# fnzhan/Neural-Gauge-Fields

Measured on AMD Instinct MI355X. Metric: Mray/sec (800x800 lego-style frame, 192 samples/ray), higher is better.
Workload: dtype f32; 1 GPU; TriPlane 800x800 frame, S=192, preset R1 (seeded random planes 256^2, dense density preset), gauge on, white_bg; samples_per_ray=192, bake_density=1, bake_color=1, launcher=none (single process)

## Files before the change

include/ngf.h:

```cpp
#ifndef NGF_H
#define NGF_H
#include <stdint.h>

#ifdef __cplusplus
extern "C" {
#endif

#define NGF_ABI_VERSION 5

enum { NGF_OK = 0, NGF_E_ARG = 1, NGF_E_HIP = 2, NGF_E_UNSUPPORTED = 3,
       NGF_E_STALE = 4  };
enum { NGF_MODEL_TRIPLANE = 0, NGF_MODEL_INFOINV = 1 };

enum {
    NGF_F_BAKE_DENSITY = 1,
    NGF_F_NO_FOLD = 4,
    NGF_F_SPLIT_BF16 = 8,
    NGF_F_BAKE_COLOR = 2
};

typedef struct ngf_field_desc {
    int32_t model;
    int32_t flags;
    int32_t plane_c;
// ... 159 lines not shown
int ngf_uv_texture_eval(const ngf_uv *m, const float *uv, const float *view, int32_t view_stride, int64_t n, int32_t flags, float *out,
                        void *hip_stream);
int ngf_uv_render(const ngf_uv *m, const float *campos_host, const float *raydir, const float *bg_host,
                  const float *jitter_u, int64_t n_rays, int32_t n_samples, float *color, float *transmittance,
                  float *dbg_sigma, float *dbg_col, uint64_t *stats, void *hip_stream);

int ngf_uv_render_batch(const ngf_uv *m, const float *campos_dev, const float *raydir, const float *bg_dev, const float *jitter_u,
                        int32_t n_cams, int64_t rays_per_cam, int32_t n_samples, float *color, float *transmittance,
                        float *dbg_sigma, float *dbg_col, uint64_t *stats, void *hip_stream);

int ngf_debug_set(const char *name, int32_t value);
int32_t ngf_debug_get(const char *name);
int ngf_debug_dirty_lds(void *hip_stream);
int ngf_debug_xcd_histogram(unsigned *out8, int32_t workgroups, void *hip_stream);
int ngf_debug_tile_plan(int64_t n, int32_t wide, int64_t resident, int32_t tail16, int64_t *seg_rays, int32_t *seg_shift);
#define NGF_UV_TRAIN_PARAMS (2 * NGF_UV_LAYERS)
typedef struct ngf_uv_train_desc {
    int32_t sphere;
    int32_t flags;
    const float *w[NGF_UV_LAYERS];
    const float *b[NGF_UV_LAYERS];
    int64_t max_rays;
    int32_t max_samples;
    int32_t pad_;
} ngf_uv_train_desc;
typedef struct ngf_uv_trainer ngf_uv_trainer;
int ngf_uv_trainer_create(const ngf_uv_train_desc *desc, ngf_uv_trainer **out, void *hip_stream);
int ngf_uv_trainer_destroy(ngf_uv_trainer *t);
int64_t ngf_uv_trainer_bytes(const ngf_uv_trainer *t);
int32_t ngf_sizeof_uv_train_desc(void);
// ... 23 lines not shown
```

neural-gauge-fields_amd/_lib.py:

```python
from __future__ import annotations

import ctypes as C
import os
import subprocess

_CSRC = os.path.join(os.path.dirname(os.path.abspath(__file__)), "csrc")
SO_PATH = os.path.join(_CSRC, "libngf_hip.so")
SO_PATH_EXP = os.path.join(_CSRC, "libngf_hip_exp.so")
_LIB = None
_LIBS = {}

MODEL_TRIPLANE, MODEL_INFOINV = 0, 1
F_BAKE_DENSITY = 1
F_BAKE_COLOR = 2
F_NO_FOLD = 4
F_SPLIT_BF16 = 8

SYMBOLS = ["ngf_field_create", "ngf_field_destroy", "ngf_field_render", "ngf_field_render_image", "ngf_field_decode_rgb", "ngf_field_march",
           "ngf_generate_rays", "ngf_generate_rays_dtu", "ngf_last_error", "ngf_abi_version", "ngf_field_bytes", "ngf_sizeof_field_desc",
           "ngf_uv_create", "ngf_uv_destroy", "ngf_uv_render", "ngf_uv_render_batch", "ngf_field_alpha", "ngf_field_ray_filter",
           "ngf_eval_workspace_bytes", "ngf_eval_frame_u8", "ngf_eval_depth_range", "ngf_eval_depth_colormap", "ngf_eval_mse",
           "ngf_eval_ssim", "ngf_trainer_create", "ngf_trainer_destroy", "ngf_trainer_bytes", "ngf_sizeof_train_desc", "ngf_train_backward", "ngf_train_backward2",
           "ngf_train_forward", "ngf_train_backward_grad", "ngf_train_get_grad", "ngf_train_get_active", "ngf_train_overflow_count", "ngf_train_adam", "ngf_train_adam_all", "ngf_train_adam_ext", "ngf_train_get_grads", "ngf_train_params_changed", "ngf_train_debug_sections", "ngf_resize_bilinear", "ngf_uv_set_texture", "ngf_uv_texture_edit", "ngf_field_alpha_mask_build", "ngf_pack_mask_bits", "ngf_debug_set", "ngf_debug_get", "ngf_debug_dirty_lds", "ngf_debug_xcd_histogram", "ngf_debug_tile_plan", "ngf_debug_tile_order", "ngf_planes_l1", "ngf_planes_l1_backward", "ngf_pool_trim", "ngf_pool_set_limit", "ngf_pool_bytes",
           "ngf_infoinv_trainer_create", "ngf_infoinv_trainer_destroy", "ngf_infoinv_trainer_bytes", "ngf_sizeof_infoinv_train_desc",
           "ngf_infoinv_train_forward", "ngf_infoinv_train_backward_grad", "ngf_infoinv_train_get_grads", "ngf_infoinv_train_params_changed",
           "ngf_infoinv_train_step_backward", "ngf_infoinv_train_set_moments", "ngf_infoinv_train_adam_all", "ngf_infoinv_train_get_grad",
           "ngf_infoinv_train_adam_ext",
           "ngf_uv_trainer_create", "ngf_uv_trainer_destroy", "ngf_uv_trainer_bytes", "ngf_sizeof_uv_train_desc", "ngf_uv_train_forward",
           "ngf_uv_train_backward", "ngf_uv_train_get_grads", "ngf_uv_train_params_changed", "ngf_uv_texture_eval"]


class FieldDesc(C.Structure):
    _fields_ = [
        ("model", C.c_int32), ("flags", C.c_int32), ("plane_c", C.c_int32), ("dens_dim", C.c_int32),
        ("plane", C.c_void_p * 3), ("plane_h", C.c_int32 * 3), ("plane_w", C.c_int32 * 3),
        ("gauge", C.c_void_p * 3), ("gauge_h", C.c_int32 * 3), ("gauge_w", C.c_int32 * 3),
        ("dens_w1", C.c_void_p), ("dens_b1", C.c_void_p), ("dens_w2", C.c_void_p),
        ("dens_b2", C.c_void_p), ("dens_w3", C.c_void_p), ("dens_b3", C.c_void_p),
# ... 70 lines not shown
        L.ngf_resize_bilinear.argtypes = [C.c_void_p, C.c_int32, C.c_int32, C.c_int32, C.c_void_p, C.c_int32, C.c_int32, C.c_void_p]
        L.ngf_eval_workspace_bytes.restype = C.c_int64
        L.ngf_eval_workspace_bytes.argtypes = [C.c_int32, C.c_int32, C.c_int32]
        L.ngf_eval_frame_u8.argtypes = [C.c_void_p, C.c_int64, C.c_void_p, C.c_void_p]
        L.ngf_eval_depth_range.argtypes = [C.c_void_p, C.c_int64, C.c_void_p, C.c_void_p, C.c_void_p]
        L.ngf_eval_depth_colormap.argtypes = [C.c_void_p, C.c_int64, C.c_void_p, C.c_void_p, C.c_void_p, C.c_void_p]
        L.ngf_eval_mse.argtypes = [C.c_void_p, C.c_void_p, C.c_int64, C.c_void_p, C.c_void_p, C.c_void_p]
        L.ngf_eval_ssim.argtypes = [C.c_void_p, C.c_void_p, C.c_int32, C.c_int32, C.c_double, C.c_int32, C.c_double, C.c_double,
                                    C.c_double, C.c_void_p, C.c_void_p, C.c_void_p, C.c_void_p]
        L.ngf_debug_set.argtypes = [C.c_char_p, C.c_int32]
        L.ngf_debug_get.argtypes = [C.c_char_p]
        L.ngf_debug_get.restype = C.c_int32
        L.ngf_debug_dirty_lds.argtypes = [C.c_void_p]
        L.ngf_debug_xcd_histogram.argtypes = [C.c_void_p, C.c_int32, C.c_void_p]
        L.ngf_debug_tile_plan.argtypes = [C.c_int64, C.c_int32, C.c_int64, C.c_int32, C.POINTER(C.c_int64), C.POINTER(C.c_int32)]
        L.ngf_pool_set_limit.argtypes = [C.c_int64]
        L.ngf_pool_bytes.argtypes = [C.c_int32]
        L.ngf_pool_bytes.restype = C.c_int64
        L.ngf_planes_l1.argtypes = [C.c_void_p, C.c_void_p, C.c_void_p, C.c_void_p, C.c_void_p]
        L.ngf_planes_l1_backward.argtypes = [C.c_void_p, C.c_void_p, C.c_void_p, C.c_void_p, C.c_void_p]
        L.ngf_debug_tile_order.argtypes = [C.c_void_p, C.c_int64, C.c_uint32, C.c_uint32, C.c_uint32, C.c_uint32, C.c_void_p]
        if L.ngf_abi_version() != 5 or L.ngf_sizeof_field_desc() != C.sizeof(FieldDesc):
            raise RuntimeError("libngf_hip.so ABI mismatch (version or ngf_field_desc layout)")
        _LIBS[path] = L
    return _LIBS[path]


class library:

    def __init__(self, which="exp"):
# ... 32 lines not shown
            check(L.ngf_debug_set(k.encode(), int(v)))
        return self

    def __exit__(self, *exc):
        L = lib()
        for k, v in self.old.items():
            L.ngf_debug_set(k.encode(), int(v))
        return False


def knobs_from_env():
    global _LIB
    if any(os.environ.get("NGF_" + k.upper()) not in (None, "", "-1") for k in ("waves", "nstep", "profile", "kernel", "stage")):
        _LIB = _load(SO_PATH_EXP)
    L = lib()
    for k in ("tile_w", "split", "waves", "nstep", "profile", "ablate", "uv_tiles", "kernel", "stage", "xcd", "grid", "tail", "ord_rows", "ord_px", "train_dwg"):
        v = os.environ.get("NGF_" + k.upper())
        check(L.ngf_debug_set(k.encode(), int(v) if v not in (None, "") else -1))
```

neural-gauge-fields_amd/csrc/ngf_device.hpp:

```cpp
#pragma once
#include <cstddef>
#include <type_traits>
#include <hip/hip_runtime.h>
#include <stdint.h>

typedef float f32x2 __attribute__((ext_vector_type(2)));
typedef float f32x4 __attribute__((ext_vector_type(4)));
typedef float f32x16 __attribute__((ext_vector_type(16)));

namespace ngf {

constexpr int kWave = 64;
constexpr int kRing = 128;
constexpr int kRecFloats = 8;
constexpr int kViewFeat = 16;

struct Tex {
    const float *p;
    int32_t W, H;
    int32_t stride;
    float fw, fh;
};

struct MaskVol {
// ... 19 lines not shown
    int32_t S, white_bg, mode, skip_rgb;
    int32_t tile_w;
    int32_t tile_shift;
    uint32_t seg_end[3];
    int32_t seg_shift[4];
    int64_t seg_ray0[4];
    int32_t xcd_queues;
    int32_t waves_active;
    uint32_t tiles;
    uint32_t ord_n;
    uint32_t ord_tpr;
    uint32_t ord_bw;
    uint32_t ord_bh;
    uint32_t queue_waves;
    int32_t ablate;
    float a0[3], a1[3], inv[3];
    float near_, far_, step, dscale, thr;
    Tex dens[3];
    Tex app[3];
    Tex gau[3];
    MaskVol mask;
    const float *basis_pack;
    const float *blob;
    int32_t blob_floats;
    float wd[48];
    float bd;
};

__device__ __forceinline__ int xcd_id() { return (int)(__builtin_amdgcn_s_getreg((3 << 11) | 20) & 7u); }

// ... 110 lines not shown
    b.wx1 = wx1; b.wy1 = wy1; b.in = in ? 1 : 0;
    wx0 = in ? wx0 : 0.0f;
    wx1 = in ? wx1 : 0.0f;
    wy0 = in ? wy0 : 0.0f;
    wy1 = in ? wy1 : 0.0f;
    b.cx = (int)cx + 1;
    b.cy = (int)cy + 1;
    b.idx = (int)__umul24((unsigned)b.cy, (unsigned)t.stride) + b.cx;
    b.w00 = wx0 * wy0;
    b.w10 = wx1 * wy0;
    b.w01 = wx0 * wy1;
    b.w11 = wx1 * wy1;
    return b;
}

template <typename T>
__device__ __forceinline__ const T *tex_at(const float *base, uint32_t float_index)
{
    return reinterpret_cast<const T *>(reinterpret_cast<const char *>(base) + (size_t)(uint32_t)(float_index * 4u));
}

__device__ __forceinline__ Bil bil_from_rec(int32_t idx, float wx1, float wy1, bool in)
{
    Bil b;
    b.idx = idx; b.cx = 0; b.cy = 0; b.wx1 = wx1; b.wy1 = wy1; b.in = in ? 1 : 0;
    float wx0 = 1.0f - wx1;
    float wy0 = 1.0f - wy1;
    wx0 = in ? wx0 : 0.0f;
    wx1 = in ? wx1 : 0.0f;
    wy0 = in ? wy0 : 0.0f;
// ... 138 lines not shown
```

neural-gauge-fields_amd/csrc/ngf_field.hip:

```cpp
#include <map>
#include <mutex>
#include <utility>

#include "ngf_host.hpp"
#include "ngf_infoinv.hpp"
#include "ngf_render.hpp"
#ifdef NGF_EXPERIMENTS
#include "ngf_render_pc.hpp"
#include "ngf_stage.hpp"
#endif
#include "ngf_train.hpp"

using namespace ngf;

static thread_local char g_err[512] = "";

int ngf::fail(int code, const char *fmt, ...)
{
    va_list ap;
    va_start(ap, fmt);
    vsnprintf(g_err, sizeof(g_err), fmt, ap);
    va_end(ap);
    return code;
}

static std::atomic<int> g_knob[ngf::KNOB_COUNT];
static const char *const g_knob_name[ngf::KNOB_COUNT] = {"tile_w", "split", "waves", "nstep", "profile", "ablate", "uv_tiles", "kernel", "stage", "poison", "grid", "xcd", "tail", "ord_rows", "ord_px", "train_dwg"};
static bool g_knob_init = [] { for (auto &k : g_knob) k.store(-1); return true; }();

int ngf::knob(int id) { return g_knob[id].load(std::memory_order_relaxed); }

hipError_t ngf::ensure_dynamic_lds(const void *kernel, size_t bytes)
{
    static std::mutex mu;
    static std::map<std::pair<int, const void *>, size_t> done;
    int dev = 0;
    hipError_t e = hipGetDevice(&dev);
    if (e != hipSuccess) return e;
    std::lock_guard<std::mutex> lock(mu);
    size_t &have = done[{dev, kernel}];
    if (have >= bytes && have != 0) return hipSuccess;
    e = hipFuncSetAttribute(kernel, hipFuncAttributeMaxDynamicSharedMemorySize, (int)bytes);
// ... 96 lines not shown
    mutable std::mutex use_mu;
    mutable std::vector<hipStream_t> streams;
    mutable std::atomic<void *> last_stream{(void *)(intptr_t)-1};
};

static inline void field_use(const ngf_field *f, hipStream_t st)
{
    if (f->last_stream.load(std::memory_order_relaxed) == (void *)st) return;
    std::lock_guard<std::mutex> lk(f->use_mu);
    bool known = false;
    for (hipStream_t s : f->streams) known |= s == st;
    if (!known) f->streams.push_back(st);
    f->last_stream.store((void *)st, std::memory_order_relaxed);
}

__global__ void pack_plane_kernel(const float *__restrict__ src, int H, int W, int c0, int nc, float *__restrict__ dst, int perm = 0)
{
    const size_t total = (size_t)(H + 2) * (W + 2) * nc;
    for (size_t i = (size_t)blockIdx.x * blockDim.x + threadIdx.x; i < total; i += (size_t)gridDim.x * blockDim.x) {
        const int c = (int)(i % nc);
        const size_t tx = i / nc;
        const int x = (int)(tx % (W + 2)), y = (int)(tx / (W + 2));
        float v = 0.0f;
        if (x >= 1 && x <= W && y >= 1 && y <= H) v = src[((size_t)(c0 + (perm ? infoinv_split_channel(c) : c)) * H + (y - 1)) * W + (x - 1)];
        dst[i] = v;
    }
}

__global__ void __launch_bounds__(256) mask_cells_kernel(const uint8_t *__restrict__ bits, int D, int H, int W, uint8_t *__restrict__ cells)
{
    ngf::MaskVol m{};
    m.bits = bits; m.D = D; m.H = H; m.W = W;
    const size_t total = (size_t)(D + 1) * (H + 1) * (W + 1);
    for (size_t i = (size_t)blockIdx.x * blockDim.x + threadIdx.x; i < total; i += (size_t)gridDim.x * blockDim.x) {
        const int x = (int)(i % (size_t)(W + 1)) - 1, y = (int)((i / (size_t)(W + 1)) % (size_t)(H + 1)) - 1, z = (int)(i / ((size_t)(W + 1) * (H + 1))) - 1;
        unsigned c = 0;
#pragma unroll
        for (int k = 0; k < 8; ++k) c |= (unsigned)ngf::mask_bit(m, z + (k >> 2), y + ((k >> 1) & 1), x + (k & 1)) << k;
        cells[i] = (uint8_t)c;
    }
}
// ... 21 lines not shown
{
    const int b = blockIdx.x * blockDim.x + threadIdx.x;
    if (b >= cD * cH * cW) return;
    const int X = b % cW, Y = (b / cW) % cH, Z = b / (cW * cH);
    unsigned acc = 0;
    for (int dz = -1; dz <= 1; ++dz)
        for (int dy = -1; dy <= 1; ++dy)
            for (int dx = -1; dx <= 1; ++dx) {
                const int x = X + dx, y = Y + dy, z = Z + dz;
                if (x >= 0 && x < cW && y >= 0 && y < cH && z >= 0 && z < cD) acc |= any[(z * cH + y) * cW + x];
            }
    clear[b] = acc ? 0 : 1;
}

__global__ void bake_density_kernel(const float *__restrict__ src, int H, int W, int nc, const float *__restrict__ wd,
                                    float *__restrict__ dst)
{
    const size_t total = (size_t)(H + 2) * (W + 2);
    for (size_t i = (size_t)blockIdx.x * blockDim.x + threadIdx.x; i < total; i += (size_t)gridDim.x * blockDim.x) {
        const int x = (int)(i % (W + 2)), y = (int)(i / (W + 2));
        double v = 0.0;
        if (x >= 1 && x <= W && y >= 1 && y <= H)
            for (int c = 0; c < nc; ++c) v += (double)wd[c] * (double)src[((size_t)c * H + (y - 1)) * W + (x - 1)];
        dst[i] = (float)v;
    }
}

__global__ void __launch_bounds__(256) bake_color_kernel(const float *__restrict__ src, int H, int W, int c0, int nc, const double *__restrict__ wp, int ldw,
                                                         float *__restrict__ dst)
{
    const size_t texels = (size_t)(H + 2) * (W + 2), plane = (size_t)H * W;
    const int lane = threadIdx.x & 63, w = __builtin_amdgcn_readfirstlane(threadIdx.x >> 6);
    const double *wr = wp + (size_t)(16 * w) * ldw;
    for (size_t t0 = (size_t)blockIdx.x * 64; t0 < texels; t0 += (size_t)gridDim.x * 64) {
        const size_t tx = t0 + lane;
        if (tx >= texels) continue;
        const int x = (int)(tx % (W + 2)), y = (int)(tx / (W + 2));
        const bool inside = x >= 1 && x <= W && y >= 1 && y <= H;
        const float *sp = src + ((size_t)c0 * H + (inside ? y - 1 : 0)) * W + (inside ? x - 1 : 0);
// ... 572 lines not shown
        return bail(fail(NGF_E_HIP, "uploading the MLP image failed"));
    A.blob = f->blob;
    A.blob_floats = (int)img.size();
    if (no_fold || split_ii) {
        if ((rc = alloc_f(&f->basis_pack, bpack.size(), f, st))) return bail(rc);
        if (hipMemcpyAsync(f->basis_pack, bpack.data(), bpack.size() * sizeof(float), hipMemcpyHostToDevice, st) != hipSuccess)
            return bail(fail(NGF_E_HIP, "uploading the packed basis matrix failed"));
        A.basis_pack = f->basis_pack;
    }
    if (tri) {
        for (int i = 0; i < 48; ++i) A.wd[i] = dw1[i];
        A.bd = db1[0];
    }

    NGF_CT("image upload");
    const int app_c = bake_c ? 64 : f->app;
    for (int p = 0; p < 3; ++p) {
        const int H = d->plane_h[p], W = d->plane_w[p];
        const size_t texels = (size_t)(H + 2) * (W + 2);
        const int dc = bake ? 1 : d->dens_dim;
        if (texels * (size_t)(app_c > 96 ? app_c : 96) * sizeof(float) >= ((size_t)1 << 32)) {
            return bail(fail(NGF_E_UNSUPPORTED, "plane %d: %d x %d texels do not fit a 4 GiB packed texture", p, H, W));
        }
        if ((rc = alloc_f(&f->tex[p], texels * dc, f, st)) || (rc = alloc_f(&f->tex[3 + p], texels * app_c, f, st))) return bail(rc);
        if (bake) bake_density_kernel<<<1024, 256, 0, st>>>(d->plane[p], H, W, d->dens_dim, d->dens_w1 + p * d->dens_dim, f->tex[p]);
        else pack_plane_kernel<<<2048, 256, 0, st>>>(d->plane[p], H, W, 0, d->dens_dim, f->tex[p]);
        if (bake_c) bake_color_kernel<<<2048, 256, 0, st>>>(d->plane[p], H, W, d->dens_dim, f->app, f->w1pd_tmp + (size_t)p * f->app, F, f->tex[3 + p]);
        else pack_plane_kernel<<<2048, 256, 0, st>>>(d->plane[p], H, W, d->dens_dim, f->app, f->tex[3 + p], tri ? 0 : 1);
        A.dens[p] = Tex{f->tex[p], W, H, W + 2, (float)(W - 1), (float)(H - 1)};
        A.app[p] = Tex{f->tex[3 + p], W, H, W + 2, (float)(W - 1), (float)(H - 1)};
        if (tri) {
            const int gh = d->gauge_h[p], gw = d->gauge_w[p];
            if ((rc = alloc_f(&f->tex[6 + p], (size_t)(gh + 2) * (gw + 2) * 2, f, st))) return bail(rc);
            pack_plane_kernel<<<256, 256, 0, st>>>(d->gauge[p], gh, gw, 0, 2, f->tex[6 + p]);
            A.gau[p] = Tex{f->tex[6 + p], gw, gh, gw + 2, (float)(gw - 1), (float)(gh - 1)};
        }
    }
    NGF_CT("texture allocs + launches");
    const bool launch_ok = hipGetLastError() == hipSuccess && hipStreamSynchronize(st) == hipSuccess;
    NGF_CT("sync (pack / bake kernels)");
    f->w1p_tmp = nullptr; f->w1pd_tmp = nullptr;
    if (!launch_ok) return bail(fail(NGF_E_HIP, "packing kernels failed"));

    for (int k = 0; k < 3; ++k) {
        A.a0[k] = d->aabb[k];
        A.a1[k] = d->aabb[3 + k];
        A.inv[k] = 2.0f / (d->aabb[3 + k] - d->aabb[k]);
    }
    A.near_ = d->near_; A.far_ = d->far_; A.step = d->step; A.dscale = d->distance_scale; A.thr = d->weight_thres;
// ... 164 lines not shown
    A.xcd_queues = knob(KNOB_XCD) > 0 ? 8 : 1;
    int64_t grid = tiles < f->num_cus ? tiles : f->num_cus;
    if (knob(KNOB_GRID) > 0 && grid > knob(KNOB_GRID)) grid = knob(KNOB_GRID);
    if (grid < 1) grid = 1;
    const int64_t per_wg = (tiles + grid - 1) / grid;
    A.waves_active = per_wg < waves ? (int)per_wg : waves;
    A.queue_waves = (uint32_t)grid;
    hipLaunchKernelGGL(k, dim3((unsigned)grid), dim3(threads), lds_bytes, st, A);
    HIP_TRY(hipGetLastError());
    return NGF_OK;
}

template <typename P>
static int launch_policy(const ngf_field *f, RenderArgs &A, hipStream_t st)
{
    const size_t lds = ((size_t)((A.blob_floats + 3) & ~3) + P::WAVES * wave_lds_floats<P>()) * sizeof(float);
    if (lds > 160 * 1024) return fail(NGF_E_ARG, "this waves-per-CU setting needs %zu bytes of LDS (> 160 KiB)", lds);
    constexpr int wide = P::INFOINV ? 16 : 8;
    using KP = decltype(&render_kernel<P, false>);
    if constexpr (P::NSTEP == 1 && P::PROD) return launch_render<KP>(render_kernel<P, false>, render_kernel<P, true>, render_kernel<P, true, false>, f, A, P::WAVES * kWave, lds, st, wide);
    else if constexpr (P::NSTEP == 1) return launch_render<KP>(render_kernel<P, false>, render_kernel<P, true>, nullptr, f, A, P::WAVES * kWave, lds, st, wide);
    else return launch_render<KP>(render_kernel<P, false>, nullptr, nullptr, f, A, P::WAVES * kWave, lds, st, wide);
}

#ifdef NGF_EXPERIMENTS
template <typename P, int NM, int NS, int TW>
static int launch_pc(const ngf_field *f, RenderArgs &A, hipStream_t st)
{
    const size_t lds = ((size_t)((A.blob_floats + 3) & ~3) + PcLds<NM>::TOTAL) * sizeof(float);
    if (lds > 160 * 1024) return fail(NGF_E_ARG, "the specialised kernel needs %zu bytes of LDS (> 160 KiB)", lds);
    const unsigned slot = f->next_counter.fetch_add(1) % kCounters;
    A.tile_counter = f->counters + (size_t)slot * kQueueHeads;
    HIP_TRY(hipMemsetAsync(A.tile_counter, 0, kQueueHeads * sizeof(unsigned), st));
    if (int rc = poison_lds(st)) return rc;
    A.xcd_queues = 1;
    A.tile_w = TW;
    A.tile_shift = TW == 8 ? 3 : 2;
    auto k = render_pc_kernel<P, NM, NS, TW>;
    HIP_TRY(ensure_dynamic_lds(reinterpret_cast<const void *>(k), lds));
    const int64_t tiles = (A.n + TW - 1) / TW;
    int64_t grid = (tiles + NM - 1) / NM;
    if (grid > f->num_cus) grid = f->num_cus;
    if (grid < 1) grid = 1;
// ... 175 lines not shown
    A.mode = mode ? 1 : 0;
    if (int rc = poison_lds(st)) return rc;
    int64_t grid = (n + 255) / 256;
    if (grid > 8 * (int64_t)f->num_cus) grid = 8 * (int64_t)f->num_cus;
    if (f->model == NGF_MODEL_INFOINV) {
        const size_t lds = (size_t)((A.blob_floats + 3) & ~3) * sizeof(float);
        if (grid > (int64_t)f->num_cus) grid = f->num_cus;
        if (f->flags & NGF_F_SPLIT_BF16) {
            HIP_TRY(ensure_dynamic_lds(reinterpret_cast<const void *>(alpha_kernel<InfoInvSplitPolicy>), lds));
            hipLaunchKernelGGL(alpha_kernel<InfoInvSplitPolicy>, dim3((unsigned)grid), dim3(256), lds, st, A, xyz, L, n, length, alpha);
        } else {
            HIP_TRY(ensure_dynamic_lds(reinterpret_cast<const void *>(alpha_kernel<InfoInvPolicy>), lds));
            hipLaunchKernelGGL(alpha_kernel<InfoInvPolicy>, dim3((unsigned)grid), dim3(256), lds, st, A, xyz, L, n, length, alpha);
        }
    } else if (f->flags & NGF_F_BAKE_DENSITY) {
        hipLaunchKernelGGL((alpha_kernel<TriPlanePolicy<true, false, 8, 1>>), dim3((unsigned)grid), dim3(256), 0, st, A, xyz, L, n, length, alpha);
    } else {
        hipLaunchKernelGGL((alpha_kernel<TriPlanePolicy<false, false, 8, 1>>), dim3((unsigned)grid), dim3(256), 0, st, A, xyz, L, n, length, alpha);
    }
    HIP_TRY(hipGetLastError());
    return NGF_OK;
}

extern "C" int ngf_field_alpha(const ngf_field *f, const float *xyz, int64_t n, int32_t mode, float length, float *alpha, void *hip_stream)
{
    if (!f || !xyz || !alpha) return fail(NGF_E_ARG, "ngf_field_alpha: null argument");
    if (n < 0) return fail(NGF_E_ARG, "ngf_field_alpha: n=%lld", (long long)n);
    if (n == 0) return NGF_OK;
    return launch_alpha(f, xyz, Lattice{nullptr, nullptr, nullptr, 0, 0, 0}, n, mode, length, alpha, (hipStream_t)hip_stream);
}

// ... 778 lines not shown
```

neural-gauge-fields_amd/csrc/ngf_host.hpp:

```cpp
#pragma once
#include <hip/hip_runtime.h>

#include <algorithm>
#include <atomic>
#include <cmath>
#include <cstdarg>
#include <chrono>
#include <cstdio>
#include <cstring>
#include <cstdlib>
#include <new>
#include <vector>

#include "../../include/ngf.h"

namespace ngf {

int fail(int code, const char *fmt, ...) __attribute__((format(printf, 2, 3)));

static constexpr int kCounters = 256;
static constexpr int kQueueHeads = 16;

enum Knob { KNOB_TILE_W = 0, KNOB_SPLIT, KNOB_WAVES, KNOB_NSTEP, KNOB_PROFILE, KNOB_ABLATE, KNOB_UV_TILES, KNOB_KERNEL, KNOB_STAGE, KNOB_POISON, KNOB_GRID, KNOB_XCD, KNOB_TAIL, KNOB_ORD_ROWS, KNOB_ORD_PX, KNOB_TRAIN_DWG, KNOB_COUNT };
int knob(int id);
hipError_t ensure_dynamic_lds(const void *kernel, size_t bytes);
constexpr unsigned kPoisonPattern = 0x7FC0DEADu;
int poison_lds(hipStream_t st);
int poison_alloc(void *p, size_t bytes, hipStream_t st);

}

#define HIP_TRY(expr)                                                                                        \
    do {                                                                                                     \
        hipError_t e_ = (expr);                                                                              \
        if (e_ != hipSuccess) return ngf::fail(NGF_E_HIP, "%s failed: %s", #expr, hipGetErrorString(e_));    \
    } while (0)

namespace ngf {
// ... 21 lines not shown
```

neural-gauge-fields_amd/csrc/ngf_render.hpp:

```cpp
#pragma once
#include <cstddef>
#include <type_traits>

#include "ngf_device.hpp"
#include "ngf_shade16.hpp"
#include "ngf_shade_bf16.hpp"

namespace ngf {


template <typename P> constexpr int wave_lds_floats() { return P::RING * kRecFloats + P::BATCH * 4 + P::VFEAT_FLOATS + P::STAGE_FLOATS; }

__device__ __forceinline__ void view_inputs(const float d[3], float v[16])
{
    v[0] = d[0]; v[1] = d[1]; v[2] = d[2];
#pragma unroll
    for (int k = 0; k < 3; ++k) {
        sincos_small(d[k], v[3 + 2 * k], v[9 + 2 * k]);
        sincos_small(d[k] * 2.0f, v[4 + 2 * k], v[10 + 2 * k]);
    }
    v[15] = 0.0f;
}

__device__ __forceinline__ void view_inputs_tile(const float d[3], float *dst, int seg, int K)
// ... 37 lines not shown
{
#pragma unroll
    for (int base = 0; base < F; base += 4) {
        float s, c;
        sincos_small(x * (float)(1 << base), s, c);
        sn[base] = s; cs[base] = c;
#pragma unroll
        for (int j = 1; j < 4 && base + j < F; ++j) {
            const float s2 = 2.0f * s * c, c2 = (c - s) * (c + s);
            s = s2; c = c2;
            sn[base + j] = s; cs[base + j] = c;
        }
    }
}

template <bool BAKED>
__device__ __forceinline__ float triplane_density_feature(const RenderArgs &A, const float t[6], Bil *cells = nullptr)
{
    float f = 0.0f;
#pragma unroll
    for (int p = 0; p < 3; ++p) {
        const Tex tx = karg_tex(offsetof(RenderArgs, dens) + p * sizeof(Tex));
        Bil b = bil_setup<BAKED>(t[2 * p], t[2 * p + 1], tx);
        if (cells) cells[p] = b;
        if (BAKED) {
            const float *q = tex_at<float>(tx.p, (uint32_t)b.idx), *q1 = tex_at<float>(tx.p, (uint32_t)(b.idx + tx.stride));
            f += bil_mix(b, q[0], q[1], q1[0], q1[1]);
        } else {
            const f32x4 *q00 = tex_at<f32x4>(tx.p, (uint32_t)b.idx * 16u);
            const f32x4 *q01 = tex_at<f32x4>(tx.p, (uint32_t)(b.idx + tx.stride) * 16u);
            float d00 = 0.0f, d10 = 0.0f, d01 = 0.0f, d11 = 0.0f;
            typedef const __attribute__((address_space(4))) float *kptr_t;
            kptr_t wdp = (kptr_t)((const __attribute__((address_space(4))) char *)__builtin_amdgcn_kernarg_segment_ptr() + offsetof(RenderArgs, wd)) + p * 16;
            asm volatile("" : "+s"(wdp));
#pragma unroll
            for (int q = 0; q < 4; ++q) {
                f32x4 v00 = q00[q], v10 = q00[4 + q], v01 = q01[q], v11 = q01[4 + q];
#pragma unroll
                for (int e = 0; e < 4; ++e) {
                    float w = wdp[4 * q + e];
                    d00 = fmaf(w, v00[e], d00);
                    d10 = fmaf(w, v10[e], d10);
                    d01 = fmaf(w, v01[e], d01);
                    d11 = fmaf(w, v11[e], d11);
                }
            }
            f += bil_mix(b, d00, d10, d01, d11);
        }
    }
    return f + A.bd;
}

template <bool MED3 = true>
__device__ __forceinline__ void triplane_gauge(const RenderArgs &A, const float x[3], int gauge_on, float t[6])
{
    const float u[3] = {x[0], x[1], x[0]}, v[3] = {x[1], x[2], x[2]};
    if (gauge_on) {
        float d[3][2];
#pragma unroll
        for (int p = 0; p < 3; ++p) {
            const Tex tx = karg_tex(offsetof(RenderArgs, gau) + p * sizeof(Tex));
            Bil b = bil_setup<MED3>(u[p], v[p], tx);
            const f32x2 *g = tex_at<f32x2>(tx.p, (uint32_t)b.idx * 2u), *g1 = tex_at<f32x2>(tx.p, (uint32_t)(b.idx + tx.stride) * 2u);
            f32x2 g00 = g[0], g10 = g[1], g01 = g1[0], g11 = g1[1];
            d[p][0] = bil_mix(b, g00[0], g10[0], g01[0], g11[0]);
            d[p][1] = bil_mix(b, g00[1], g10[1], g01[1], g11[1]);
        }
        t[0] = (u[0] + d[0][0]) + d[2][0];  t[1] = (v[0] + d[0][1]) + d[1][0];
        t[2] = (u[1] + d[1][0]) + d[0][1];  t[3] = (v[1] + d[1][1]) + d[2][1];
        t[4] = (u[2] + d[2][0]) + d[0][0];  t[5] = (v[2] + d[2][1]) + d[1][1];
    } else {
#pragma unroll
        for (int p = 0; p < 3; ++p) { t[2 * p] = u[p]; t[2 * p + 1] = v[p]; }
    }
}

template <bool BAKE_D, bool BAKE_C, int WAVES_, int NSTEP_, bool PROFILE_ = false>
struct TriPlanePolicy {
    static constexpr bool PROFILE = PROFILE_;
    static constexpr bool PROD = WAVES_ == 12 && NSTEP_ == 1 && !PROFILE_;
    static constexpr bool INFOINV = false;
    static constexpr bool MASK_SKIP = false;
    static constexpr bool STAGED = false;
    static constexpr int STAGE_FLOATS = 0;
    static constexpr int WAVES = WAVES_;
    static constexpr int NSTEP = NSTEP_;
    static constexpr int BATCH = kBatch16;
    static constexpr bool VLDS = WAVES_ <= 12;
    static constexpr int VFEAT_FLOATS = VLDS ? kWave * kViewFeat : 0;
    static constexpr int RING = NSTEP_ == 1 ? 128 : 256;
    static constexpr bool REC12 = WAVES_ == 12 && NSTEP_ == 1 && !PROFILE_;
    static constexpr bool GATHER_QUAD = BAKE_C;
    __device__ static __forceinline__ float sigma(const RenderArgs &A, const float *, bool valid, const float x[3], int, float t[6], Bil *cells = nullptr)
    {
        float tt[6];
        triplane_gauge<BAKE_D>(A, x, A.mode, tt);
        const float sg = softplus_shift(triplane_density_feature<BAKE_D>(A, tt, cells));
#pragma unroll
        for (int k = 0; k < 6; ++k) t[k] = valid ? tt[k] : 0.0f;
        return valid ? sg : 0.0f;
    }
    static constexpr bool VIEW_FOLD = VLDS;
    __device__ static __forceinline__ void fold_view(const float *smem, const float *vfeat, float *pre, int n_rays, int lane)
    {
        if constexpr (BAKE_C) view_fold16<MlpLayout16Baked::W1V / 64, MlpLayout16Baked::B1, 4>(per_pass16(smem), vfeat, pre, n_rays, lane);
        else view_fold16<MlpLayout16<48>::W1 / 64 + 3 * MlpLayout16<48>::QCH, MlpLayout16<48>::B1, MlpLayout16<48>::KT>(per_pass16(smem), vfeat, pre, n_rays, lane);
    }
    __device__ static __forceinline__ void fold_view_regs(const float *smem, const f32x4 v, float *pre, int n_rays, int lane)
    {
        if constexpr (BAKE_C) view_fold16_regs<MlpLayout16Baked::W1V / 64, MlpLayout16Baked::B1, 4>(per_pass16(smem), v, pre, n_rays, lane);
        else view_fold16_regs<MlpLayout16<48>::W1 / 64 + 3 * MlpLayout16<48>::QCH, MlpLayout16<48>::B1, MlpLayout16<48>::KT>(per_pass16(smem), v, pre, n_rays, lane);
    }
    __device__ static __forceinline__ void shade(const RenderArgs &A, const float *smem, const float rec[kRecFloats], const float *vf,
                                                 const float od[3], int lane, float c[3], unsigned long long *tk = nullptr, const float *pre = nullptr)
    {
// ... 9 lines not shown
        f32x4 v = {0.0f, 0.0f, 0.0f, 0.0f};
        if (!pre) v = *reinterpret_cast<const f32x4 *>(vf + (lane >> 4) * 4);
        if constexpr (BAKE_C) mlp_pass16_baked(A, smem, rec, v, lane, c, pre, &cells);
        else mlp_pass16<48>(A, smem, rec, v, lane, c, nullptr, pre, &cells);
    }
};

template <typename P>
struct MaskSkip : P {
#ifdef NGF_EXP_NO_MASK_SKIP
    static constexpr bool MASK_SKIP = false;
#else
    static constexpr bool MASK_SKIP = true;
#endif
};

template <bool BAKE_D, int WAVES_ = 8>
struct TriPlaneBf16Policy : TriPlanePolicy<BAKE_D, false, WAVES_, 1> {
    static constexpr bool PROD = WAVES_ == 8;
    static constexpr bool REC12 = false;
    static constexpr bool VIEW_FOLD = false;
    static constexpr int VFEAT_FLOATS = 8 * kViewFeat;
    __device__ static __forceinline__ void shade(const RenderArgs &A, const float *smem, const float rec[kRecFloats], const float *vf,
                                                 const float od[3], int lane, float c[3], unsigned long long * = nullptr, const float * = nullptr)
    {
        const f32x4 v = *reinterpret_cast<const f32x4 *>(vf + (lane >> 4) * 4);
        if constexpr (WAVES_ > 8) mlp_pass16_bf16_rows(A, smem, rec, v, lane, c);
        else mlp_pass16_bf16(A, smem, rec, v, lane, c);
    }
};
// ... 667 lines not shown
```

Before: 147.3 Mray/s.

## Pack baked density and gauge planes as row pairs for single-fetch bilinear taps

Repacks the baked density plane and the gauge planes so each texel also stores the texel one row below it. The four bilinear taps then come from one contiguous vector load instead of two loads from separate rows. When all three gauge planes share one resolution, the per-axis bilinear setup is computed once per coordinate and reused across planes. This doubles the memory footprint of those planes and adds template variants (GaugeAny) for the case where gauge resolutions differ.

```diff
diff --git a/include/ngf.h b/include/ngf.h
--- a/include/ngf.h
+++ b/include/ngf.h
@@ -197,6 +197,7 @@
 int ngf_debug_dirty_lds(void *hip_stream);
 int ngf_debug_xcd_histogram(unsigned *out8, int32_t workgroups, void *hip_stream);
 int ngf_debug_tile_plan(int64_t n, int32_t wide, int64_t resident, int32_t tail16, int64_t *seg_rays, int32_t *seg_shift);
+int64_t ngf_debug_packed_plane_floats(int32_t H, int32_t W, int32_t nc, int32_t pair);
 #define NGF_UV_TRAIN_PARAMS (2 * NGF_UV_LAYERS)
 typedef struct ngf_uv_train_desc {
     int32_t sphere;
diff --git a/neural-gauge-fields_amd/_lib.py b/neural-gauge-fields_amd/_lib.py
--- a/neural-gauge-fields_amd/_lib.py
+++ b/neural-gauge-fields_amd/_lib.py
@@ -21,7 +21,7 @@
            "ngf_uv_create", "ngf_uv_destroy", "ngf_uv_render", "ngf_uv_render_batch", "ngf_field_alpha", "ngf_field_ray_filter",
            "ngf_eval_workspace_bytes", "ngf_eval_frame_u8", "ngf_eval_depth_range", "ngf_eval_depth_colormap", "ngf_eval_mse",
            "ngf_eval_ssim", "ngf_trainer_create", "ngf_trainer_destroy", "ngf_trainer_bytes", "ngf_sizeof_train_desc", "ngf_train_backward", "ngf_train_backward2",
-           "ngf_train_forward", "ngf_train_backward_grad", "ngf_train_get_grad", "ngf_train_get_active", "ngf_train_overflow_count", "ngf_train_adam", "ngf_train_adam_all", "ngf_train_adam_ext", "ngf_train_get_grads", "ngf_train_params_changed", "ngf_train_debug_sections", "ngf_resize_bilinear", "ngf_uv_set_texture", "ngf_uv_texture_edit", "ngf_field_alpha_mask_build", "ngf_pack_mask_bits", "ngf_debug_set", "ngf_debug_get", "ngf_debug_dirty_lds", "ngf_debug_xcd_histogram", "ngf_debug_tile_plan", "ngf_debug_tile_order", "ngf_planes_l1", "ngf_planes_l1_backward", "ngf_pool_trim", "ngf_pool_set_limit", "ngf_pool_bytes",
+           "ngf_train_forward", "ngf_train_backward_grad", "ngf_train_get_grad", "ngf_train_get_active", "ngf_train_overflow_count", "ngf_train_adam", "ngf_train_adam_all", "ngf_train_adam_ext", "ngf_train_get_grads", "ngf_train_params_changed", "ngf_train_debug_sections", "ngf_resize_bilinear", "ngf_uv_set_texture", "ngf_uv_texture_edit", "ngf_field_alpha_mask_build", "ngf_pack_mask_bits", "ngf_debug_set", "ngf_debug_get", "ngf_debug_dirty_lds", "ngf_debug_xcd_histogram", "ngf_debug_tile_plan", "ngf_debug_packed_plane_floats", "ngf_debug_tile_order", "ngf_planes_l1", "ngf_planes_l1_backward", "ngf_pool_trim", "ngf_pool_set_limit", "ngf_pool_bytes",
            "ngf_infoinv_trainer_create", "ngf_infoinv_trainer_destroy", "ngf_infoinv_trainer_bytes", "ngf_sizeof_infoinv_train_desc",
            "ngf_infoinv_train_forward", "ngf_infoinv_train_backward_grad", "ngf_infoinv_train_get_grads", "ngf_infoinv_train_params_changed",
            "ngf_infoinv_train_step_backward", "ngf_infoinv_train_set_moments", "ngf_infoinv_train_adam_all", "ngf_infoinv_train_get_grad",
@@ -122,6 +122,8 @@
         L.ngf_debug_dirty_lds.argtypes = [C.c_void_p]
         L.ngf_debug_xcd_histogram.argtypes = [C.c_void_p, C.c_int32, C.c_void_p]
         L.ngf_debug_tile_plan.argtypes = [C.c_int64, C.c_int32, C.c_int64, C.c_int32, C.POINTER(C.c_int64), C.POINTER(C.c_int32)]
+        L.ngf_debug_packed_plane_floats.argtypes = [C.c_int32, C.c_int32, C.c_int32, C.c_int32]
+        L.ngf_debug_packed_plane_floats.restype = C.c_int64
         L.ngf_pool_set_limit.argtypes = [C.c_int64]
         L.ngf_pool_bytes.argtypes = [C.c_int32]
         L.ngf_pool_bytes.restype = C.c_int64
@@ -184,6 +186,6 @@
     if any(os.environ.get("NGF_" + k.upper()) not in (None, "", "-1") for k in ("waves", "nstep", "profile", "kernel", "stage")):
         _LIB = _load(SO_PATH_EXP)
     L = lib()
-    for k in ("tile_w", "split", "waves", "nstep", "profile", "ablate", "uv_tiles", "kernel", "stage", "xcd", "grid", "tail", "ord_rows", "ord_px", "train_dwg"):
+    for k in ("tile_w", "split", "waves", "nstep", "profile", "ablate", "uv_tiles", "kernel", "stage", "xcd", "grid", "tail", "ord_rows", "ord_px", "train_dwg", "pairpack"):
         v = os.environ.get("NGF_" + k.upper())
         check(L.ngf_debug_set(k.encode(), int(v) if v not in (None, "") else -1))
diff --git a/neural-gauge-fields_amd/csrc/ngf_device.hpp b/neural-gauge-fields_amd/csrc/ngf_device.hpp
--- a/neural-gauge-fields_amd/csrc/ngf_device.hpp
+++ b/neural-gauge-fields_amd/csrc/ngf_device.hpp
@@ -7,6 +7,7 @@
 typedef float f32x2 __attribute__((ext_vector_type(2)));
 typedef float f32x4 __attribute__((ext_vector_type(4)));
 typedef float f32x16 __attribute__((ext_vector_type(16)));
+typedef float f32x4_a8 __attribute__((ext_vector_type(4), aligned(8)));
 
 namespace ngf {
 
@@ -57,6 +58,8 @@
     uint32_t ord_bh;
     uint32_t queue_waves;
     int32_t ablate;
+    int32_t gauge_same;
+    int32_t pairpack;
     float a0[3], a1[3], inv[3];
     float near_, far_, step, dscale, thr;
     Tex dens[3];
@@ -197,6 +200,40 @@
     return b;
 }
 
+struct BilAxis {
+    float w0, w1;
+    int32_t c;
+    bool in;
+};
+__device__ __forceinline__ BilAxis bil_axis(float u, float fw)
+{
+    const float px = ((u + 1.0f) / 2.0f) * fw;
+    const float fx = floorf(px);
+    BilAxis a;
+    a.w1 = px - fx; a.w0 = 1.0f - a.w1;
+    const float cx = __builtin_amdgcn_fmed3f(fx, -1.0f, fw);
+    a.in = cx == fx;
+#ifdef NGF_EXP_NOMASK
+    a.in = true;
+#endif
+    a.c = (int)cx + 1;
+    return a;
+}
+__device__ __forceinline__ Bil bil_from_axes(const BilAxis &x, const BilAxis &y, int32_t stride)
+{
+    const bool in = x.in & y.in;
+    Bil b;
+    b.wx1 = x.w1; b.wy1 = y.w1; b.in = in ? 1 : 0;
+    const float wx0 = in ? x.w0 : 0.0f, wx1 = in ? x.w1 : 0.0f, wy0 = in ? y.w0 : 0.0f, wy1 = in ? y.w1 : 0.0f;
+    b.cx = x.c; b.cy = y.c;
+    b.idx = (int)__umul24((unsigned)y.c, (unsigned)stride) + x.c;
+    b.w00 = wx0 * wy0;
+    b.w10 = wx1 * wy0;
+    b.w01 = wx0 * wy1;
+    b.w11 = wx1 * wy1;
+    return b;
+}
+
 template <typename T>
 __device__ __forceinline__ const T *tex_at(const float *base, uint32_t float_index)
 {
diff --git a/neural-gauge-fields_amd/csrc/ngf_field.hip b/neural-gauge-fields_amd/csrc/ngf_field.hip
--- a/neural-gauge-fields_amd/csrc/ngf_field.hip
+++ b/neural-gauge-fields_amd/csrc/ngf_field.hip
@@ -25,7 +25,7 @@
 }
 
 static std::atomic<int> g_knob[ngf::KNOB_COUNT];
-static const char *const g_knob_name[ngf::KNOB_COUNT] = {"tile_w", "split", "waves", "nstep", "profile", "ablate", "uv_tiles", "kernel", "stage", "poison", "grid", "xcd", "tail", "ord_rows", "ord_px", "train_dwg"};
+static const char *const g_knob_name[ngf::KNOB_COUNT] = {"tile_w", "split", "waves", "nstep", "profile", "ablate", "uv_tiles", "kernel", "stage", "poison", "grid", "xcd", "tail", "ord_rows", "ord_px", "train_dwg", "pairpack"};
 static bool g_knob_init = [] { for (auto &k : g_knob) k.store(-1); return true; }();
 
 int ngf::knob(int id) { return g_knob[id].load(std::memory_order_relaxed); }
@@ -152,7 +152,7 @@
     f->last_stream.store((void *)st, std::memory_order_relaxed);
 }
 
-__global__ void pack_plane_kernel(const float *__restrict__ src, int H, int W, int c0, int nc, float *__restrict__ dst, int perm = 0)
+__global__ void pack_plane_kernel(const float *__restrict__ src, int H, int W, int c0, int nc, float *__restrict__ dst, int perm = 0, int pair = 0)
 {
     const size_t total = (size_t)(H + 2) * (W + 2) * nc;
     for (size_t i = (size_t)blockIdx.x * blockDim.x + threadIdx.x; i < total; i += (size_t)gridDim.x * blockDim.x) {
@@ -161,8 +161,20 @@
         const int x = (int)(tx % (W + 2)), y = (int)(tx / (W + 2));
         float v = 0.0f;
         if (x >= 1 && x <= W && y >= 1 && y <= H) v = src[((size_t)(c0 + (perm ? infoinv_split_channel(c) : c)) * H + (y - 1)) * W + (x - 1)];
-        dst[i] = v;
-    }
+        if (pair) {
+            dst[tx * 2 * nc + c] = v;
+            if (y >= 1) dst[((tx - (W + 2)) * 2 + 1) * nc + c] = v;
+            if (y == H + 1) dst[(tx * 2 + 1) * nc + c] = 0.0f;
+        } else dst[i] = v;
+    }
+}
+
+static inline size_t packed_plane_floats(int H, int W, int nc, bool pair) { return (size_t)(H + 2) * (W + 2) * nc * (pair ? 2 : 1); }
+
+extern "C" int64_t ngf_debug_packed_plane_floats(int32_t H, int32_t W, int32_t nc, int32_t pair)
+{
+    if (H < 1 || W < 1 || nc < 1) return -1;
+    return (int64_t)packed_plane_floats(H, W, nc, pair != 0);
 }
 
 __global__ void __launch_bounds__(256) mask_cells_kernel(const uint8_t *__restrict__ bits, int D, int H, int W, uint8_t *__restrict__ cells)
@@ -214,7 +226,7 @@
 }
 
 __global__ void bake_density_kernel(const float *__restrict__ src, int H, int W, int nc, const float *__restrict__ wd,
-                                    float *__restrict__ dst)
+                                    float *__restrict__ dst, int pair)
 {
     const size_t total = (size_t)(H + 2) * (W + 2);
     for (size_t i = (size_t)blockIdx.x * blockDim.x + threadIdx.x; i < total; i += (size_t)gridDim.x * blockDim.x) {
@@ -222,7 +234,11 @@
         double v = 0.0;
         if (x >= 1 && x <= W && y >= 1 && y <= H)
             for (int c = 0; c < nc; ++c) v += (double)wd[c] * (double)src[((size_t)c * H + (y - 1)) * W + (x - 1)];
-        dst[i] = (float)v;
+        if (pair) {
+            dst[i * 2] = (float)v;
+            if (y >= 1) dst[(i - (W + 2)) * 2 + 1] = (float)v;
+            if (y == H + 1) dst[i * 2 + 1] = 0.0f;
+        } else dst[i] = (float)v;
     }
 }
 
@@ -825,6 +841,18 @@
     }
 
     NGF_CT("image upload");
+    bool pair = bake;
+#ifdef NGF_EXPERIMENTS
+    if (knob(KNOB_PAIRPACK) == 0) pair = false;
+#else
+    if (knob(KNOB_PAIRPACK) == 0) return bail(fail(NGF_E_UNSUPPORTED, "knob pairpack = 0 (the one-row layout of the march's planes) exists in libngf_hip_exp.so only"));
+#endif
+    A.pairpack = pair ? 1 : 0;
+    A.gauge_same = 0;
+    if (tri && bake) {
+        A.gauge_same = 1;
+        for (int p = 0; p < 3; ++p) A.gauge_same &= d->gauge_h[p] == d->gauge_w[0] && d->gauge_w[p] == d->gauge_w[0];
+    }
     const int app_c = bake_c ? 64 : f->app;
     for (int p = 0; p < 3; ++p) {
         const int H = d->plane_h[p], W = d->plane_w[p];
@@ -833,8 +861,8 @@
         if (texels * (size_t)(app_c > 96 ? app_c : 96) * sizeof(float) >= ((size_t)1 << 32)) {
             return bail(fail(NGF_E_UNSUPPORTED, "plane %d: %d x %d texels do not fit a 4 GiB packed texture", p, H, W));
         }
-        if ((rc = alloc_f(&f->tex[p], texels * dc, f, st)) || (rc = alloc_f(&f->tex[3 + p], texels * app_c, f, st))) return bail(rc);
-        if (bake) bake_density_kernel<<<1024, 256, 0, st>>>(d->plane[p], H, W, d->dens_dim, d->dens_w1 + p * d->dens_dim, f->tex[p]);
+        if ((rc = alloc_f(&f->tex[p], packed_plane_floats(H, W, dc, pair), f, st)) || (rc = alloc_f(&f->tex[3 + p], texels * app_c, f, st))) return bail(rc);
+        if (bake) bake_density_kernel<<<1024, 256, 0, st>>>(d->plane[p], H, W, d->dens_dim, d->dens_w1 + p * d->dens_dim, f->tex[p], pair ? 1 : 0);
         else pack_plane_kernel<<<2048, 256, 0, st>>>(d->plane[p], H, W, 0, d->dens_dim, f->tex[p]);
         if (bake_c) bake_color_kernel<<<2048, 256, 0, st>>>(d->plane[p], H, W, d->dens_dim, f->app, f->w1pd_tmp + (size_t)p * f->app, F, f->tex[3 + p]);
         else pack_plane_kernel<<<2048, 256, 0, st>>>(d->plane[p], H, W, d->dens_dim, f->app, f->tex[3 + p], tri ? 0 : 1);
@@ -842,8 +870,8 @@
         A.app[p] = Tex{f->tex[3 + p], W, H, W + 2, (float)(W - 1), (float)(H - 1)};
         if (tri) {
             const int gh = d->gauge_h[p], gw = d->gauge_w[p];
-            if ((rc = alloc_f(&f->tex[6 + p], (size_t)(gh + 2) * (gw + 2) * 2, f, st))) return bail(rc);
-            pack_plane_kernel<<<256, 256, 0, st>>>(d->gauge[p], gh, gw, 0, 2, f->tex[6 + p]);
+            if ((rc = alloc_f(&f->tex[6 + p], packed_plane_floats(gh, gw, 2, pair), f, st))) return bail(rc);
+            pack_plane_kernel<<<256, 256, 0, st>>>(d->gauge[p], gh, gw, 0, 2, f->tex[6 + p], 0, pair ? 1 : 0);
             A.gau[p] = Tex{f->tex[6 + p], gw, gh, gw + 2, (float)(gw - 1), (float)(gh - 1)};
         }
     }
@@ -1038,6 +1066,9 @@
 template <typename P>
 static int launch_policy(const ngf_field *f, RenderArgs &A, hipStream_t st)
 {
+    if constexpr (shared_gauge<P>::value) {
+        if (!A.gauge_same) return launch_policy<GaugeAny<P>>(f, A, st);
+    }
     const size_t lds = ((size_t)((A.blob_floats + 3) & ~3) + P::WAVES * wave_lds_floats<P>()) * sizeof(float);
     if (lds > 160 * 1024) return fail(NGF_E_ARG, "this waves-per-CU setting needs %zu bytes of LDS (> 160 KiB)", lds);
     constexpr int wide = P::INFOINV ? 16 : 8;
@@ -1051,6 +1082,9 @@
 template <typename P, int NM, int NS, int TW>
 static int launch_pc(const ngf_field *f, RenderArgs &A, hipStream_t st)
 {
+    if constexpr (shared_gauge<P>::value) {
+        if (!A.gauge_same) return launch_pc<GaugeAny<P>, NM, NS, TW>(f, A, st);
+    }
     const size_t lds = ((size_t)((A.blob_floats + 3) & ~3) + PcLds<NM>::TOTAL) * sizeof(float);
     if (lds > 160 * 1024) return fail(NGF_E_ARG, "the specialised kernel needs %zu bytes of LDS (> 160 KiB)", lds);
     const unsigned slot = f->next_counter.fetch_add(1) % kCounters;
@@ -1256,7 +1290,8 @@
             hipLaunchKernelGGL(alpha_kernel<InfoInvPolicy>, dim3((unsigned)grid), dim3(256), lds, st, A, xyz, L, n, length, alpha);
         }
     } else if (f->flags & NGF_F_BAKE_DENSITY) {
-        hipLaunchKernelGGL((alpha_kernel<TriPlanePolicy<true, false, 8, 1>>), dim3((unsigned)grid), dim3(256), 0, st, A, xyz, L, n, length, alpha);
+        if (A.gauge_same) hipLaunchKernelGGL((alpha_kernel<TriPlanePolicy<true, false, 8, 1>>), dim3((unsigned)grid), dim3(256), 0, st, A, xyz, L, n, length, alpha);
+        else hipLaunchKernelGGL((alpha_kernel<GaugeAny<TriPlanePolicy<true, false, 8, 1>>>), dim3((unsigned)grid), dim3(256), 0, st, A, xyz, L, n, length, alpha);
     } else {
         hipLaunchKernelGGL((alpha_kernel<TriPlanePolicy<false, false, 8, 1>>), dim3((unsigned)grid), dim3(256), 0, st, A, xyz, L, n, length, alpha);
     }
diff --git a/neural-gauge-fields_amd/csrc/ngf_host.hpp b/neural-gauge-fields_amd/csrc/ngf_host.hpp
--- a/neural-gauge-fields_amd/csrc/ngf_host.hpp
+++ b/neural-gauge-fields_amd/csrc/ngf_host.hpp
@@ -21,7 +21,7 @@
 static constexpr int kCounters = 256;
 static constexpr int kQueueHeads = 16;
 
-enum Knob { KNOB_TILE_W = 0, KNOB_SPLIT, KNOB_WAVES, KNOB_NSTEP, KNOB_PROFILE, KNOB_ABLATE, KNOB_UV_TILES, KNOB_KERNEL, KNOB_STAGE, KNOB_POISON, KNOB_GRID, KNOB_XCD, KNOB_TAIL, KNOB_ORD_ROWS, KNOB_ORD_PX, KNOB_TRAIN_DWG, KNOB_COUNT };
+enum Knob { KNOB_TILE_W = 0, KNOB_SPLIT, KNOB_WAVES, KNOB_NSTEP, KNOB_PROFILE, KNOB_ABLATE, KNOB_UV_TILES, KNOB_KERNEL, KNOB_STAGE, KNOB_POISON, KNOB_GRID, KNOB_XCD, KNOB_TAIL, KNOB_ORD_ROWS, KNOB_ORD_PX, KNOB_TRAIN_DWG, KNOB_PAIRPACK, KNOB_COUNT };
 int knob(int id);
 hipError_t ensure_dynamic_lds(const void *kernel, size_t bytes);
 constexpr unsigned kPoisonPattern = 0x7FC0DEADu;
diff --git a/neural-gauge-fields_amd/csrc/ngf_render.hpp b/neural-gauge-fields_amd/csrc/ngf_render.hpp
--- a/neural-gauge-fields_amd/csrc/ngf_render.hpp
+++ b/neural-gauge-fields_amd/csrc/ngf_render.hpp
@@ -75,16 +75,20 @@
     }
 }
 
-template <bool BAKED>
+template <bool BAKED, bool PAIR = false>
 __device__ __forceinline__ float triplane_density_feature(const RenderArgs &A, const float t[6], Bil *cells = nullptr)
 {
+    static_assert(BAKED || !PAIR, "only the 1-channel baked density planes have a row-pair form");
     float f = 0.0f;
 #pragma unroll
     for (int p = 0; p < 3; ++p) {
         const Tex tx = karg_tex(offsetof(RenderArgs, dens) + p * sizeof(Tex));
         Bil b = bil_setup<BAKED>(t[2 * p], t[2 * p + 1], tx);
         if (cells) cells[p] = b;
-        if (BAKED) {
+        if (BAKED && PAIR) {
+            const f32x4_a8 q = *tex_at<f32x4_a8>(tx.p, (uint32_t)b.idx * 2u);
+            f += bil_mix(b, q[0], q[2], q[1], q[3]);
+        } else if (BAKED) {
             const float *q = tex_at<float>(tx.p, (uint32_t)b.idx), *q1 = tex_at<float>(tx.p, (uint32_t)(b.idx + tx.stride));
             f += bil_mix(b, q[0], q[1], q1[0], q1[1]);
         } else {
@@ -112,20 +116,43 @@
     return f + A.bd;
 }
 
-template <bool MED3 = true>
+template <bool MED3 = true, bool PAIR = false, bool SAME = false>
 __device__ __forceinline__ void triplane_gauge(const RenderArgs &A, const float x[3], int gauge_on, float t[6])
 {
     const float u[3] = {x[0], x[1], x[0]}, v[3] = {x[1], x[2], x[2]};
     if (gauge_on) {
         float d[3][2];
-#pragma unroll
-        for (int p = 0; p < 3; ++p) {
-            const Tex tx = karg_tex(offsetof(RenderArgs, gau) + p * sizeof(Tex));
-            Bil b = bil_setup<MED3>(u[p], v[p], tx);
-            const f32x2 *g = tex_at<f32x2>(tx.p, (uint32_t)b.idx * 2u), *g1 = tex_at<f32x2>(tx.p, (uint32_t)(b.idx + tx.stride) * 2u);
-            f32x2 g00 = g[0], g10 = g[1], g01 = g1[0], g11 = g1[1];
+        auto fetch = [&](int p, const Tex &tx, const Bil &b) {
+            f32x2 g00, g10, g01, g11;
+            if constexpr (PAIR) {
+                const f32x4 *g = tex_at<f32x4>(tx.p, (uint32_t)b.idx * 4u);
+                const f32x4 a = g[0], c = g[1];
+                g00 = f32x2{a[0], a[1]}; g01 = f32x2{a[2], a[3]}; g10 = f32x2{c[0], c[1]}; g11 = f32x2{c[2], c[3]};
+            } else {
+                const f32x2 *g = tex_at<f32x2>(tx.p, (uint32_t)b.idx * 2u), *g1 = tex_at<f32x2>(tx.p, (uint32_t)(b.idx + tx.stride) * 2u);
+                g00 = g[0]; g10 = g[1]; g01 = g1[0]; g11 = g1[1];
+            }
             d[p][0] = bil_mix(b, g00[0], g10[0], g01[0], g11[0]);
             d[p][1] = bil_mix(b, g00[1], g10[1], g01[1], g11[1]);
+        };
+        if constexpr (PAIR && MED3 && SAME) {
+            const Tex t0 = karg_tex(offsetof(RenderArgs, gau));
+            BilAxis ax[3];
+#pragma unroll
+            for (int k = 0; k < 3; ++k) ax[k] = bil_axis(x[k], t0.fw);
+            const int ua[3] = {0, 1, 0}, va[3] = {1, 2, 2};
+#pragma unroll
+            for (int p = 0; p < 3; ++p) {
+                Tex tx = t0;
+                tx.p = karg<const float *>(offsetof(RenderArgs, gau) + p * sizeof(Tex) + offsetof(Tex, p));
+                fetch(p, tx, bil_from_axes(ax[ua[p]], ax[va[p]], t0.stride));
+            }
+        } else {
+#pragma unroll
+            for (int p = 0; p < 3; ++p) {
+                const Tex tx = karg_tex(offsetof(RenderArgs, gau) + p * sizeof(Tex));
+                fetch(p, tx, bil_setup<MED3>(u[p], v[p], tx));
+            }
         }
         t[0] = (u[0] + d[0][0]) + d[2][0];  t[1] = (v[0] + d[0][1]) + d[1][0];
         t[2] = (u[1] + d[1][0]) + d[0][1];  t[3] = (v[1] + d[1][1]) + d[2][1];
@@ -152,14 +179,30 @@
     static constexpr int RING = NSTEP_ == 1 ? 128 : 256;
     static constexpr bool REC12 = WAVES_ == 12 && NSTEP_ == 1 && !PROFILE_;
     static constexpr bool GATHER_QUAD = BAKE_C;
-    __device__ static __forceinline__ float sigma(const RenderArgs &A, const float *, bool valid, const float x[3], int, float t[6], Bil *cells = nullptr)
+    static constexpr bool SHARED_GAUGE = BAKE_D;
+    template <bool SAME>
+    __device__ static __forceinline__ float sigma_impl(const RenderArgs &A, bool valid, const float x[3], float t[6], Bil *cells)
     {
         float tt[6];
-        triplane_gauge<BAKE_D>(A, x, A.mode, tt);
-        const float sg = softplus_shift(triplane_density_feature<BAKE_D>(A, tt, cells));
+        float f;
+#ifdef NGF_EXPERIMENTS
+        if (BAKE_D && !A.pairpack) {
+            triplane_gauge<BAKE_D, false>(A, x, A.mode, tt);
+            f = triplane_density_feature<BAKE_D, false>(A, tt, cells);
+        } else
+#endif
+        {
+            triplane_gauge<BAKE_D, BAKE_D, SAME>(A, x, A.mode, tt);
+            f = triplane_density_feature<BAKE_D, BAKE_D>(A, tt, cells);
+        }
+        const float sg = softplus_shift(f);
 #pragma unroll
         for (int k = 0; k < 6; ++k) t[k] = valid ? tt[k] : 0.0f;
         return valid ? sg : 0.0f;
+    }
+    __device__ static __forceinline__ float sigma(const RenderArgs &A, const float *, bool valid, const float x[3], int, float t[6], Bil *cells = nullptr)
+    {
+        return sigma_impl<true>(A, valid, x, t, cells);
     }
     static constexpr bool VIEW_FOLD = VLDS;
     __device__ static __forceinline__ void fold_view(const float *smem, const float *vfeat, float *pre, int n_rays, int lane)
@@ -199,6 +242,17 @@
     static constexpr bool MASK_SKIP = true;
 #endif
 };
+
+template <typename P>
+struct GaugeAny : P {
+    static constexpr bool SHARED_GAUGE = false;
+    __device__ static __forceinline__ float sigma(const RenderArgs &A, const float *, bool valid, const float x[3], int, float t[6], Bil *cells = nullptr)
+    {
+        return P::template sigma_impl<false>(A, valid, x, t, cells);
+    }
+};
+template <typename P, typename = void> struct shared_gauge : std::false_type {};
+template <typename P> struct shared_gauge<P, std::void_t<decltype(P::SHARED_GAUGE)>> : std::integral_constant<bool, P::SHARED_GAUGE> {};
 
 template <bool BAKE_D, int WAVES_ = 8>
 struct TriPlaneBf16Policy : TriPlanePolicy<BAKE_D, false, WAVES_, 1> {
```

New measurement: 150.0 Mray/s, median of 6. +1.8%, better.
